# eleurent/rl-agents

Measured on AMD Instinct MI355X. Metric: rollout env-steps/sec (UCT plan(), budget=1000), higher is better.
Workload: dtype f64; 1 GPU; uct_highway_shaped_S10000_A5_budget1000_e33xh30_roots262144_per_gpu; n_roots_per_gpu=262144, n_roots_total=262144, states=10000, actions=5, episodes=33, horizon=30, parallelism=roots sharded over 1 GPU(s)

## Files before the change

### rl_agents_amd/csrc/common.hpp

```cpp
#pragma once
#include <hip/hip_runtime.h>
#include <stdint.h>
#include <stdio.h>
#include <string>
#include <unordered_map>
#include <vector>

#include "../../include/mi355plan.h"
#include "form_names.hpp"

namespace mp {

constexpr int kWave = 64;
constexpr size_t kLdsBytes = 160 * 1024;

extern thread_local std::string g_err;

int fail(int code, const char *fmt, ...);

#define MP_HIP(call)                                                                              \
    do {                                                                                          \
        hipError_t e_ = (call);                                                                   \
        if (e_ != hipSuccess)                                                                     \
            return mp::fail(MP_ERR_HIP, "%s failed: %s (%s:%d)", #call, hipGetErrorString(e_),    \
                            __FILE__, __LINE__);                                                  \
    } while (0)

#define MP_TRY(call)                  \
    do {                              \
        int rc_ = (call);             \
        if (rc_ != MP_OK) return rc_; \
    } while (0)

struct alignas(16) Rec {
    int32_t next;
    uint32_t flags;
    double reward;
};
static_assert(sizeof(Rec) == 16, "Rec must be one dwordx4");

struct DevBuf {
    void *p = nullptr;
    size_t cap = 0;
};

struct TreeMeta {
    int kind = 0;
    int n_roots = 0, A = 0, cap = 0, K = 0, M = 1;
    double gamma = 0.0;
    int buf = 0;
    bool armed = false;
    int il = 0;
    long kept_bound = 0;
    bool virgin = false;
    bool sp = false;
    int n_src = 0;
};

enum { WS_TREE0 = 0, WS_TREE1, WS_TREE2, WS_TREE3, WS_TREE4, WS_TREE5, WS_TREE6, WS_TREE7, WS_IO0, WS_IO1, WS_IO2, WS_IO3, WS_IO4,
       WS_IO5, WS_IO6, WS_IO7, WS_IO8, WS_IO9, WS_TAB0, WS_TAB1, WS_TAB2, WS_TAB3, WS_VI0, WS_VI1, WS_VI2, WS_VI3,
       WS_VI4, WS_VI5, WS_GROOT, WS_JUMP, WS_POL0, WS_POL1, WS_POL2, WS_POL3, WS_POL4,
       WS_IO10,
       WS_COUNT };

struct ViGraphKey {
    const void *model, *T, *R, *term, *Vb, *notclose;
    int iterations, M, S, A, robust, vform;
    double gamma, rtol, atol;
};

}

struct mp_ctx {
    int device = 0;
    hipStream_t stream = nullptr;
    bool own_stream = false;
    hipEvent_t ev0 = nullptr, ev1 = nullptr;
    bool timed = false;
    int n_launches = 0;
    char last_variant[mp::kFormNameBytes] = "";
    hipDeviceProp_t prop;
    mp::DevBuf ws[mp::WS_COUNT];
    mp::TreeMeta tree;
    std::vector<double> tab_host;
    int tab_kind = 0;
    void *vi_graph_exec = nullptr;
    mp::ViGraphKey vi_graph_key;
// ... 249 lines not shown
```

### rl_agents_amd/csrc/uct.hip

```cpp
#include <limits.h>
#include <math.h>
#include <stdlib.h>
#include <string.h>

#include <algorithm>
#include <new>
#include <vector>

#include <type_traits>

#include "common.hpp"
#include "libm_sincos.hpp"
#include "pcg64.hpp"
#include "uct_balance.hpp"
#include "uct_host.hpp"
#include "uct_virgin.hpp"
#include "wave.hpp"

namespace mp {

struct alignas(16) UctNode {
    double value;
    int32_t count;
    int32_t first_child;
// ... 107 lines not shown
    const double temp = (force + polemass_length * (theta_dot * theta_dot) * sintheta) / total_mass;
    const double thetaacc = (c.gravity * sintheta - costheta * temp) /
                            (c.length * (4.0 / 3.0 - c.masspole * (costheta * costheta) / total_mass));
    const double xacc = temp - polemass_length * thetaacc * costheta / total_mass;
    x = x + c.tau * x_dot;
    x_dot = x_dot + c.tau * xacc;
    theta = theta + c.tau * theta_dot;
    theta_dot = theta_dot + c.tau * thetaacc;
    x4[0] = x; x4[1] = x_dot; x4[2] = theta; x4[3] = theta_dot;
    return x < -c.x_threshold || x > c.x_threshold || theta < -c.theta_threshold || theta > c.theta_threshold;
}

__device__ __forceinline__ uint32_t bal_load(const uint32_t *w) { return __hip_atomic_load(w, __ATOMIC_RELAXED, __HIP_MEMORY_SCOPE_WORKGROUP); }
__device__ __forceinline__ void bal_store(uint32_t *w, uint32_t v) { __hip_atomic_store(w, v, __ATOMIC_RELAXED, __HIP_MEMORY_SCOPE_WORKGROUP); }

__device__ __forceinline__ uint32_t simd_id()
{
    uint32_t v;
    asm volatile("s_getreg_b32 %0, hwreg(HW_REG_HW_ID, 4, 2)" : "=s"(v));
    return v;
}
#ifdef MP_WAVE_STAMPS
constexpr int kWaveStampWords = 8;
#endif

enum { ENV_TABLE = 0, ENV_CARTPOLE = 2, ENV_TABLE_LDSR = 3, ENV_TABLE_SPILL = 4 };

#ifndef MP_UCT_MIN_WAVES
#define MP_UCT_MIN_WAVES 1
#endif
#ifndef MP_PCG_WORDS
#define MP_PCG_WORDS 1
#endif
constexpr bool uct_pcg_words_form(int AT, int ENV, bool SP, bool MK, int IL, bool QD)
{
    return ENV != ENV_CARTPOLE && !QD;
}
template <int AT, int ENV, bool SP = false, bool MK = false, int IL = 0, bool QD = false, bool BAL = false>
__global__ __launch_bounds__(ENV == ENV_TABLE_LDSR ? 1024 : (ENV == ENV_CARTPOLE ? 256 : 64),
                             ENV == ENV_TABLE_LDSR ? 1 : (SP && AT > 0 && AT <= 5 && MP_UCT_MIN_WAVES < 4 ? 4 : MP_UCT_MIN_WAVES))
void uct_kernel(UctArgs p)
{
    static_assert(!SP || (AT > 0 && ENV == ENV_TABLE), "per-state policies: table env, |A| known at compile time");
    static_assert(!MK || SP, "listed policies are per-state policies");
    constexpr int NTH = AT > 1 ? AT - 1 : 1;
    constexpr int NQ = (NTH + 1) / 2;
    constexpr int NQ32 = (NTH + 3) / 4;
    constexpr bool LDSR = ENV == ENV_TABLE_LDSR;
    static_assert(!LDSR || (AT > 0 && !SP), "the LDS-resident variant: |A| at compile time, state-independent policies");
    static_assert(!QD || LDSR, "four lanes per root: the LDS-resident model");
    constexpr bool PREG = LDSR || ENV == ENV_TABLE_SPILL;
    constexpr bool CART = ENV == ENV_CARTPOLE;
    constexpr bool RAWU = AT > 0 && !SP;
    constexpr int USH = RAWU ? 0 : 11;
    static_assert(!BAL || (LDSR && !QD), "the wave balance: the one-lane LDS-resident form");
    extern __shared__ __attribute__((aligned(16))) double lds_raw[];
    extern __shared__ __attribute__((aligned(16))) uint32_t lds_bal[];
    double *lds_d = lds_raw + (BAL ? kUctBalBytes / sizeof(double) : 0);
    const int tid = threadIdx.x, lane = tid & 63, wave = tid >> 6;
    const int A = AT > 0 ? AT : p.A, H = p.horizon, E = p.episodes;
    const int nthreads = p.waves * 64;
    double *gpow = lds_d;
    const uint64_t *thr = reinterpret_cast<const uint64_t *>(gpow + (H + 1));
    double *tp = gpow + (H + 1) + A;
    const int TE = p.table_n;
    double *rcp = tp + A;
    double *tpdiv = rcp + (TE + 1);
    const int ntab = (H + 1) + 2 * A + (TE + 1) + A * (TE + 2);
    auto explore = [&](int a, int cnt1) { return cnt1 <= TE + 1 ? tpdiv[a * (TE + 2) + cnt1] : tp[a] / (double)cnt1; };
    auto inv = [&](int c) { return c <= TE ? rcp[c] : 1.0 / (double)c; };
    auto explore_tab = [&](int a, int cnt1) { return tpdiv[a * (TE + 2) + min(cnt1, TE + 1)]; };
// ... 36 lines not shown
        const uint4 *src = reinterpret_cast<const uint4 *>(p.r8);
        uint4 *dst = reinterpret_cast<uint4 *>(r8);
        for (int i = tid; i < n16; i += nthreads) dst[i] = src[i];
    }
    if (LDSR) {
        const int n = p.S * A;
        const int n8 = n >> 3;
        const uint4 *src = reinterpret_cast<const uint4 *>(p.t16);
        uint4 *dst = reinterpret_cast<uint4 *>(t16);
        for (int i = tid; i < n8; i += nthreads) dst[i] = src[i];
        for (int i = (n8 << 3) + tid; i < n; i += nthreads) t16[i] = p.t16[i];
    }
    if constexpr (BAL) {
        const int g0 = blockIdx.x * p.waves + wave;
        const uint32_t mine = (long)g0 * p.lanes < p.n_roots ? uct_bal_word(0, simd_id()) : kUctBalGone;
        if (lane < kUctBalWords && ((lane ^ g0) & (p.waves - 1)) == 0) bal_store(&lds_bal[lane], lane == (g0 & (kUctBalWords - 1)) ? mine : kUctBalGone);
    }
    __syncthreads();
    WAVE_STAMP(1);
    int32_t *path = path_all + wave * 64;
    const int slot = QD ? lane >> 2 : (CART ? lane >> p.rep_shift : lane);
    const bool owner = QD ? (lane & 3) == 0 : true;
    const int r = (blockIdx.x * p.waves + wave) * p.lanes + slot;
#ifdef MP_WAVE_STAMPS
    if (slot >= p.lanes || r >= p.n_roots) { WAVE_STAMP(2); WAVE_STAMP(3); }
#endif
    if (slot >= p.lanes || r >= p.n_roots) return;
    static_assert(IL != 2 || AT > 0, "the group-interleaved layout needs |A| at compile time");
    const TreeRef<IL, AT> tree = tree_of<IL, AT>(p.tree, r, p.cap, A);
    constexpr bool WEXP = IL == 2 && AT > 0 && AT <= 5 && !MK && !LDSR && !CART;
    constexpr int WEXP_PASSES = 4;
    constexpr bool LEAF1 = AT > 0 && !(LDSR && !QD && AT >= 7);
    const bool leaf1 = LEAF1 && p.tree_stores != 0;
    constexpr bool VSKIP = uct_virgin_form(AT, ENV, SP, MK, IL, QD);
    constexpr bool VDEFER = VSKIP && LEAF1;
    const bool vskip = VSKIP && p.tree_stores == 2;
    const bool vdefer = VDEFER && p.tree_stores == 2 && p.n_nodes_in == nullptr;
    bool wave_exp = false;
    if constexpr (WEXP) {
        const int wave_r0 = (blockIdx.x * p.waves + __builtin_amdgcn_readfirstlane(wave)) * 64;
        wave_exp = p.tree_stores != 0 && p.lanes == 64 && wave_r0 + 64 <= p.n_roots;
    }
    const Rec *__restrict__ rec = p.rec;
    Pcg64 g;
    g.load(p.rng + (long)r * 6);
    constexpr bool PCGW = MP_PCG_WORDS != 0 && uct_pcg_words_form(AT, ENV, SP, MK, IL, QD);
    using RollGen = typename std::conditional<PCGW, Pcg64W, Pcg64>::type;
    auto roll_gen = [](const Pcg64 &x) { if constexpr (PCGW) return Pcg64W::from(x); else return x; };
    auto roll_gen_commit = [](Pcg64 &x, const RollGen &y) { if constexpr (PCGW) y.state_to(x); else x = y; };
    uint64_t g4_lo = 0, g4_hi = 0;
    if (QD || (CART && p.rep_shift >= 2)) g.inc_g4(g4_lo, g4_hi);
    uint64_t g16_lo = 0, g16_hi = 0;
    if (CART && p.rep_shift >= 4) g.inc_g16(g16_lo, g16_hi);
    const int32_t s0 = CART ? 0 : p.root_state[r];
    const int32_t st0 = p.root_steps ? p.root_steps[r] : 0;
    const uint32_t done_bit = p.done_on_next ? 2u : 1u;
    const bool root_term = CART ? false : (rec[(long)s0 * A].flags & 1u) != 0;
    double x0[4] = {0.0, 0.0, 0.0, 0.0};
    if (CART) {
#pragma unroll
        for (int i = 0; i < 4; ++i) x0[i] = p.root_x[(long)r * 4 + i];
    }
    const bool cart_flat = CART && p.cp_sincos != SINCOS_DEVICE && p.cp.theta_threshold < 0.8 && !any64(!(fabs(x0[2]) < 0.8));
    int n_nodes = p.n_nodes_in ? p.n_nodes_in[r] : 0;
    constexpr int AR = AT > 0 ? AT : 1;
    constexpr bool RC = AT > 0;
    double tv0 = 0.0, tv[AR];
    int tc0 = 0, tc[AR];
    int tf0 = -1, tf[AR];
// ... 52 lines not shown
            if (pd_ >= 2 + KEEP) hh_ = p.path_spill[(size_t)pd_ * p.spill_stride + r];          \
            out_ = hh_;                                                                         \
        }                                                                                       \
    } while (0)

    constexpr int TREE_PRIO = LDSR && !QD ? 2 : 0;
#ifdef MP_PROFILE
    long long t_sel = 0, t_expd = 0, t_roll = 0, t_bak = 0, n_sel = 0, n_roll = 0;
    const long long t_all0 = clock64();
#define PROF_T(x) const long long x = clock64()
#else
#define PROF_T(x)
#endif
    for (int ep = 0; ep < E; ++ep) {
        PROF_T(c0);
        if constexpr (TREE_PRIO > 0) __builtin_amdgcn_s_setprio(TREE_PRIO);
        int32_t s = s0, st = st0;
        double x4[4] = {x0[0], x0[1], x0[2], x0[3]};
        int node = 0, depth = 0;
        bool terminal = false;
        bool cur_term = root_term;
        double total = 0.0;
        uint32_t cur_mask = mask0;
        if (!RC) PATH_PUT(0, tree.root_handle());
        int hnode = tree.root_handle();
        int fc = RC ? tf0 : tree[0].first_child;
        const bool beyond = RC && any64(tc0 >= TE);
        int node_c = 0;
        while (owner && depth < H && fc >= 0 && !terminal) {
            int act = 0, nfc = -1;
            if (AT > 0) {
                UctNode c[AR];
                bool virgin = false;
                if (fc == 1) {
#pragma unroll
                    for (int a = 0; a < AR; ++a) { c[a].value = tv[a]; c[a].count = tc[a]; c[a].first_child = tf[a]; }
                } else if (VSKIP && vskip && node_c == 1) {
                    virgin = true;
#pragma unroll
                    for (int a = 0; a < AR; ++a) { c[a].value = 0.0; c[a].count = 0; c[a].first_child = -1; }
                } else {
                    UctNode *grp = &tree.child(fc, 0);
#pragma unroll
                    for (int a = 0; a < AR; ++a) c[a] = tree.sibling(grp, a);
                }
                double sc[AR];
                if (SP) {
                    double tpl[AR];
                    if (depth == 0) {
#pragma unroll
                        for (int a = 0; a < AR; ++a) tpl[a] = tp0[a];
                    } else {
                        const double *pr = p.pol_prior + (long)s * p.pol_stride;
                        const double TAk = MK ? p.temperature * (double)__popc(cur_mask) : p.TA;
#pragma unroll
                        for (int a = 0; a < AR; ++a) tpl[a] = TAk * pr[a];
                    }
#pragma unroll
                    for (int a = 0; a < AR; ++a) {
                        sc[a] = c[a].value + tpl[a] / (double)(c[a].count + 1);
                        if (MK && c[a].count < 0) sc[a] = -INFINITY;
                    }
                } else {
                    double ex[AR];
#pragma unroll
                    for (int a = 0; a < AR; ++a) ex[a] = explore_tab(a, c[a].count + 1);
                    if (beyond) {
#pragma nounroll
                        for (int b = 0; b < AR; ++b) {
// ... 9 lines not shown
                    for (int a = 0; a < AR; ++a) sc[a] = c[a].value + ex[a];
                }
                double m = sc[0];
#pragma unroll
                for (int a = 1; a < AR; ++a) m = sc[a] > m ? sc[a] : m;
                int nt = 0;
#pragma unroll
                for (int a = 0; a < AR; ++a) nt += sc[a] == m ? 1 : 0;
                int pick = nt > 1 ? (int)g.below((uint32_t)nt) : 0;
                bool found = false;
                double sel_v = 0.0;
                int sel_c = 0;
#pragma unroll
                for (int a = 0; a < AR; ++a) {
                    const bool eq = sc[a] == m;
                    if (eq && !found && pick == 0) {
                        act = a; nfc = c[a].first_child; found = true;
                        sel_v = c[a].value; sel_c = c[a].count;
                    }
                    if (eq && !found) --pick;
                }
#pragma unroll
                for (int i = 0; i < KEEP; ++i)
                    if (depth + 1 == 2 + i) { kv[i] = sel_v; kc[i] = sel_c; }
                node_c = sel_c;
                if (VDEFER && vdefer && virgin) {
                    UctNode z;
                    z.value = 0.0; z.count = 0; z.first_child = -1;
                    UctNode *grp = &tree.child(fc, 0);
                    const bool deep = depth + 1 >= 2 + KEEP;
#pragma unroll
                    for (int a = 0; a < AR; ++a)
                        if (a != act || deep) tree.sibling(grp, a) = z;
                }
            } else {
                double m = 0.0;
                for (int a = 0; a < A; ++a) {
                    const UctNode c = tree.child(fc, a);
                    const double sc = c.value + explore(a, c.count + 1);
                    if (a == 0 || sc > m) m = sc;
                }
                int nt = 0;
                for (int a = 0; a < A; ++a) {
                    const UctNode c = tree.child(fc, a);
                    nt += (c.value + explore(a, c.count + 1)) == m ? 1 : 0;
                }
                int pick = (int)g.below((uint32_t)nt);
                for (int a = 0; a < A; ++a) {
                    const UctNode c = tree.child(fc, a);
                    if ((c.value + explore(a, c.count + 1)) == m) {
                        if (pick == 0) { act = a; nfc = c.first_child; break; }
                        --pick;
                    }
                }
            }
            const long idx = (long)s * A + act;
            double reward;
            if (CART) {
                terminal = cartpole_step(p.cp, x4, act, p.cp_sincos, sctab);
                reward = 1.0;
            } else if (LDSR) {
                const uint32_t e = t16[idx];
                reward = rdict[r8[idx]];
                const bool next_term = (e & 0x8000u) != 0;
                terminal = p.done_on_next ? next_term : cur_term;
                cur_term = next_term;
// ... 16 lines not shown
            node = fc + act;
            hnode = tree.handle(fc, act);
            ++depth;
            PATH_PUT(depth, hnode);
            fc = nfc;
#ifdef MP_PROFILE
            ++n_sel;
#endif
        }
        PROF_T(c1);
        bool wexp_pend = false;
        if (owner && fc < 0 && depth < H && (!terminal || node == 0)) {
            UctNode n;
            n.value = 0.0; n.count = 0; n.first_child = -1;
            if (RC && node <= A) {
                if (node == 0) tf0 = n_nodes;
#pragma unroll
                for (int a = 0; a < AR; ++a) tf[a] = node == 1 + a ? n_nodes : tf[a];
            } else if (!leaf1) {
                tree.at(hnode).first_child = n_nodes;
            }
            if (LEAF1) fc = n_nodes;
            if (MK) {
                if (node == 0) {
#pragma unroll
                    for (int a = 0; a < AR; ++a) tc[a] = (cur_mask >> a) & 1u ? 0 : -1;
                } else {
                    UctNode *grp = &tree.child(n_nodes, 0);
                    for (int a = 0; a < A; ++a) {
                        n.count = (cur_mask >> a) & 1u ? 0 : -1;
                        tree.sibling(grp, a) = n;
                    }
                }
            } else if (VDEFER && vdefer) {
            } else if (!(RC && node == 0)) {
                if constexpr (WEXP) {
                    wexp_pend = true;
                } else {
                    UctNode *grp = &tree.child(n_nodes, 0);
                    if (AT > 0) {
#pragma unroll
                        for (int a = 0; a < AR; ++a) tree.sibling(grp, a) = n;
                    } else {
                        for (int a = 0; a < A; ++a) tree.sibling(grp, a) = n;
                    }
                }
            }
            n_nodes += A;
        }
        if constexpr (WEXP) {
            UctNode n;
            n.value = 0.0; n.count = 0; n.first_child = -1;
            const int grp_id = n_nodes - AT;
            if (wave_exp) {
                unsigned long long rem = ballot64(wexp_pend);
                for (int pass = 0; pass < WEXP_PASSES && rem != 0ull; ++pass) {
                    const int v = __builtin_amdgcn_readlane(grp_id, __ffsll((long long)rem) - 1);
                    const bool mine = wexp_pend && grp_id == v;
                    const unsigned long long M = ballot64(mine);
                    const uint32_t m_lo = (uint32_t)M, m_hi = (uint32_t)(M >> 32);
                    const int ln = (int)__builtin_amdgcn_mbcnt_hi(~0u, __builtin_amdgcn_mbcnt_lo(~0u, 0u));
                    UctNode *run = tree.base - ln * AT + (unsigned)((v - 1 + AT) << 6);
#pragma nounroll
                    for (int i = 0; i < AT; ++i) {
                        const unsigned e = (unsigned)(i * 64 + ln), q = e / (unsigned)AT;
                        if ((((q & 32u) ? m_hi : m_lo) >> (q & 31u)) & 1u) run[e] = n;
                    }
// ... 556 lines not shown
                    n -= tree.handle(1, 0);
                    double v = tv[0];
                    int cnt = tc[0];
#pragma unroll
                    for (int a = 1; a < AR; ++a) { v = n == a ? tv[a] : v; cnt = n == a ? tc[a] : cnt; }
                    cnt += 1;
                    v += inv_fast(cnt) * (total - v);
#pragma unroll
                    for (int a = 0; a < AR; ++a) { tv[a] = n == a ? v : tv[a]; tc[a] = n == a ? cnt : tc[a]; }
                }
                tc0 += 1;
                tv0 += inv_fast(tc0) * (total - tv0);
            }
        }
#ifdef MP_PROFILE
        { const long long c4 = clock64(); t_sel += c1 - c0; t_expd += c2 - c1; t_roll += c3 - c2; t_bak += c4 - c3; }
#endif
    }
    if constexpr (BAL) {
        if ((((uint32_t)r) & 63u) == 0u) bal_store(&lds_bal[((uint32_t)r >> 6) & (kUctBalWords - 1)], kUctBalGone);
    }
    WAVE_STAMP(2);
    if constexpr (TREE_PRIO > 0) __builtin_amdgcn_s_setprio(0);
#ifdef MP_PROFILE
    if (r == 0)
        printf("uct prof wave0: total=%lld select=%lld expand=%lld rollout=%lld backup=%lld | lane0 select steps=%lld rollout steps=%lld\n",
               (long long)(clock64() - t_all0), t_sel, t_expd, t_roll, t_bak, n_sel, n_roll);
#endif
    if (!owner) return;
    if (CART && (lane & ((1 << p.rep_shift) - 1)) != 0) return;
    if (RC) {
        UctNode w;
        w.value = tv0; w.count = tc0; w.first_child = tf0;
        tree[0] = w;
        if (tf0 == 1) {
#pragma unroll
            for (int a = 0; a < AR; ++a) {
                w.value = tv[a]; w.count = tc[a]; w.first_child = tf[a];
                tree.child(1, a) = w;
            }
        }
    }
    g.store(p.rng + (long)r * 6);
    {
        int len = 0;
        int fc = tree[0].first_child;
        int at_c = 0;
        while (fc >= 0) {
            if (VDEFER && vdefer && at_c == 1) {
                if (p.plans && len < p.max_plan_len) p.plans[(long)r * p.max_plan_len + len] = 0;
                ++len;
                break;
            }
            int mc = tree.child(fc, 0).count;
            for (int a = 1; a < A; ++a) mc = max(mc, tree.child(fc, a).count);
            int best = -1;
            double bv = 0.0;
            for (int a = 0; a < A; ++a) {
                const UctNode c = tree.child(fc, a);
                if (c.count == mc && (best < 0 || c.value > bv)) { best = a; bv = c.value; }
            }
            if (p.plans && len < p.max_plan_len) p.plans[(long)r * p.max_plan_len + len] = best;
            ++len;
            at_c = tree.child(fc, best).count;
            fc = tree.child(fc, best).first_child;
        }
        if (p.plans)
            for (int i = len; i < p.max_plan_len; ++i) p.plans[(long)r * p.max_plan_len + i] = -1;
        if (p.plan_len) p.plan_len[r] = len;
    }
    if (p.n_nodes_out) p.n_nodes_out[r] = n_nodes;
    if (p.root_value) p.root_value[r] = tree[0].value;
    if (p.env_steps) p.env_steps[r] = (int64_t)steps_taken;
    const int rfc = tree[0].first_child;
    for (int a = 0; a < A; ++a) {
        if (p.root_child_count) p.root_child_count[(long)r * A + a] = rfc >= 0 ? max(tree.child(rfc, a).count, 0) : 0;
        if (p.root_child_value) p.root_child_value[(long)r * A + a] = rfc >= 0 ? tree.child(rfc, a).value : 0.0;
    }
    WAVE_STAMP(3);
#undef WAVE_STAMP
}

template <int AT, bool EACH = false, bool MW = false>
__global__ __launch_bounds__(EACH ? 256 : 1024, EACH ? 4 : 1) void uct_lone_kernel(UctArgs p)
{
    static_assert(!(EACH && MW), "one MDP per root is staged per workgroup: one root each");
    static_assert(AT >= 2 && AT <= 8, "|A| with a compile-time specialisation");
    constexpr int A = AT, NTH = AT - 1;
    extern __shared__ __attribute__((aligned(16))) double lds_d[];
    const int tid = threadIdx.x, lane = tid & 63, nthreads = blockDim.x;
    const int H = p.horizon, E = p.episodes, TE = p.table_n;
    double *gpow = lds_d;
    double *tp = gpow + (H + 1) + A;
    double *rcp = tp + A;
    double *tpdiv = rcp + (TE + 1);
    const int ntab = (H + 1) + 2 * A + (TE + 1) + A * (TE + 2);
    const int ntab2 = (ntab + 1) & ~1;
    const int SA = (EACH ? p.Sb : p.S) * A;
    const double *rdict = lds_d + ntab2;
    double *rew = lds_d + ntab2;
    uint16_t *t16 = EACH ? reinterpret_cast<uint16_t *>(rew + ((SA + 1) & ~1))
                         : reinterpret_cast<uint16_t *>(lds_d + ntab2 + (MW ? 0 : ((p.n_rdict + 1) & ~1)));
    uint8_t *r8 = reinterpret_cast<uint8_t *>(t16 + ((SA + 7) & ~7));
    uint32_t *jump0 = (EACH || MW) ? reinterpret_cast<uint32_t *>(r8) : reinterpret_cast<uint32_t *>(r8 + ((SA + 15) & ~15));
    const int W = MW ? p.waves : 1;
    const int wstride = ((H + 5) * 8 + p.cap * 6 + 3) & ~3;
    uint32_t *jump = jump0 + (MW ? (tid >> 6 < W ? tid >> 6 : 0) * wstride : 0);
// ... 629 lines not shown
            int mc = tnode[fc].count;
            for (int a = 1; a < A; ++a) mc = max(mc, tnode[fc + a].count);
            int best = -1;
            double bv = 0.0;
            for (int a = 0; a < A; ++a) {
                const UctNode c = tnode[fc + a];
                if (c.count == mc && (best < 0 || c.value > bv)) { best = a; bv = c.value; }
            }
            if (p.plans && len < p.max_plan_len) p.plans[(long)r * p.max_plan_len + len] = best;
            ++len;
            fc = tnode[fc + best].first_child;
        }
        if (p.plans)
            for (int i = len; i < p.max_plan_len; ++i) p.plans[(long)r * p.max_plan_len + i] = -1;
        if (p.plan_len) p.plan_len[r] = len;
        if (p.n_nodes_out) p.n_nodes_out[r] = n_nodes;
        if (p.root_value) p.root_value[r] = tnode[0].value;
        if (p.env_steps) p.env_steps[r] = (int64_t)steps_taken;
        const int rfc = tnode[0].first_child;
        for (int a = 0; a < A; ++a) {
            if (p.root_child_count) p.root_child_count[(long)r * A + a] = rfc >= 0 ? max(tnode[rfc + a].count, 0) : 0;
            if (p.root_child_value) p.root_child_value[(long)r * A + a] = rfc >= 0 ? tnode[rfc + a].value : 0.0;
        }
    }
}

template <int IL>
__global__ void uct_path_count_kernel(UctNode *trees, int root, int cap, int A, const int32_t *actions, int n, int64_t *out, int virgin)
{
    const TreeRef<IL, 0> tree = tree_of<IL, 0>(trees, root, cap, A);
    int node = 0;
    bool unstored = false;
    for (int i = 0; i < n; ++i) {
        const int fc = unstored ? -1 : tree[node].first_child;
        const int a = actions[i];
        if (fc < 0 || a < 0 || a >= A) { out[0] = -1; return; }
        unstored = virgin && tree[node].count == 1;
        node = fc + a;
    }
    const int c = unstored ? 0 : tree[node].count;
    out[0] = c < 0 ? -1 : c;
}

template <int IL>
__global__ __launch_bounds__(64) void uct_reroot_kernel(int n_roots, int n_src, int A, int cap_old, int cap_new,
                                                        const UctNode *__restrict__ old_trees, UctNode *__restrict__ new_trees,
                                                        const int32_t *n_old, const int32_t *__restrict__ source,
                                                        const int32_t *__restrict__ actions,
                                                        int32_t *n_new,
                                                        int virgin)
{
    const int r = blockIdx.x * blockDim.x + threadIdx.x;
    if (r >= n_roots) return;
    const int q = source ? source[r] : r;
    if (q < 0 || q >= n_src) {
        n_new[r] = 0;
        return;
    }
    const TreeRef<IL, 0> o = tree_of<IL, 0>(const_cast<UctNode *>(old_trees), q, cap_old, A);
    const TreeRef<IL, 0> n = tree_of<IL, 0>(new_trees, r, cap_new, A);
    const int a = actions[r];
    if (n_old[q] < 1 || o[0].first_child < 0 || a < 0 || a >= A || o[o[0].first_child + a].count < 0) {
        n_new[r] = 0;
        return;
    }
    int head = 0, tail = 1;
    UctNode first;
    first.first_child = o[0].first_child + a;
    n[0] = first;
    while (head < tail) {
        const int oid = n[head].first_child;
        UctNode src;
        src.value = 0.0; src.count = 0; src.first_child = -1;
        if (oid >= 0) src = o[oid];
        UctNode out;
        out.value = src.value; out.count = src.count; out.first_child = -1;
        if (src.first_child >= 0) {
            out.first_child = tail;
            const bool unstored = virgin && src.count == 1;
            for (int c = 0; c < A; ++c) {
                UctNode q;
                q.value = 0.0; q.count = 0; q.first_child = unstored ? -2 : src.first_child + c;
                n[tail + c] = q;
            }
            tail += A;
        }
        n[head] = out;
        ++head;
    }
    n_new[r] = tail;
}

struct PolBuild {
    int S, A, stride, frq, rows, shift, can_pack;
    const double *prior, *rollout;
    const uint8_t *listed, *slot;
    const Rec *rec;
    double *hp;
    uint64_t *ht;
    uint32_t *lmask;
    uint32_t *hf, *hfr, *hp16;
    int32_t *err;
};
__device__ __forceinline__ void pol_err(const PolBuild &b, int code, int s)
{
    if (atomicCAS(b.err, 0, code) == 0) b.err[1] = s;
}
__global__ void policy_rows_kernel(PolBuild b)
{
    const int s = blockIdx.x * blockDim.x + threadIdx.x;
    if (s >= b.S) return;
    const int A = b.A, r = s % b.rows;
    double cdf[8];
    double acc = 0.0;
    unsigned seen = 0;
// ... 38 lines not shown
        const uint64_t hi = t53 >> b.shift;
        f[4 + a] = hi > 0xffffffffULL ? 0xffffffffu : (uint32_t)hi;
        if (b.can_pack && a < 4) th[a] = (t53 >> 43) > 1023ULL ? 1023u : (uint32_t)(t53 >> 43);
    }
    if (b.can_pack) {
        uint32_t *g = b.hp16 + (size_t)i * 4;
        g[0] = (uint32_t)nx | (th[0] << 20);
        g[1] = (rc.y & 3u) | (th[1] << 2) | (th[2] << 12) | (th[3] << 22);
        g[2] = rc.z; g[3] = rc.w;
    }
}
__global__ void policy_froll_kernel(PolBuild b)
{
    const long i = (long)blockIdx.x * blockDim.x + threadIdx.x;
    if (i >= (long)b.S * b.A) return;
    const int s = (int)(i / b.A), k = (int)(i % b.A), r = s % b.rows;
    const int c = b.slot[(size_t)r * b.A + k];
    if (c >= b.A) return;
    const uint4 *src = reinterpret_cast<const uint4 *>(b.hf) + ((size_t)s * b.A + c) * b.frq;
    uint4 *dst = reinterpret_cast<uint4 *>(b.hfr) + (size_t)i * b.frq;
    for (int q = 0; q < b.frq; ++q) dst[q] = src[q];
}

}

using namespace mp;

static int uct_reroot_now(mp_ctx *ctx, long cap_new)
{
    const int n_roots = ctx->tree.n_roots;
    const int old_slot = ctx->tree.buf ? WS_TREE2 : WS_TREE0, new_slot = ctx->tree.buf ? WS_TREE0 : WS_TREE2;
    UctNode *nw = nullptr;
    MP_TRY(ws_get(ctx, new_slot, (size_t)((n_roots + 63) & ~63) * tree_stride_alloc(ctx->tree.il, cap_new, ctx->tree.A), &nw));
    const int virgin = ctx->tree.virgin ? 1 : 0;
    ctx->tree.virgin = false;
    return reroot_apply(ctx, cap_new, [&](const Reroot &r) {
        hipLaunchKernelGGL(ctx->tree.il == 2 ? uct_reroot_kernel<2> : uct_reroot_kernel<0>, dim3((unsigned)((r.n_roots + 63) / 64)), dim3(64), 0,
                           ctx->stream, r.n_roots, r.n_src, r.A, r.cap_old, r.cap_new, (const UctNode *)ctx->ws[old_slot].p, nw, r.sizes, r.src,
                           r.acts, r.sizes_new, virgin);
    });
}

enum UctForm { UF_GLOBAL, UF_GLOBAL_SPILL, UF_LDSR, UF_QUAD, UF_LONE, UF_LONE_MW, UF_LONE_EACH, UF_ROW_EACH, UF_ROW_SHARED,
               UF_CARTPOLE, UF_POLICY, UF_COUNT };
static_assert(UF_COUNT == kUctForms, "uct_form_name (form_names.hpp) names the forms in this order");

constexpr int kUnset = INT_MIN;
struct UctKnobs {
    int model;
    int quad, lone, each, row, rows;
    int lone_waves;
    int row_waves, row_roots, lanes, cart_rep, cart_waves;
    int path;
    long ldsr_waves;
    int tree_stores;
    int balance;
};
static int uct_knob(const char *name)
{
    const char *e = getenv(name);
    return e ? atoi(e) : kUnset;
}
static UctKnobs uct_knobs_read()
{
    UctKnobs k;
    const char *model = getenv("MP_UCT_MODEL"), *path = getenv("MP_UCT_PATH"), *ldsr_waves = getenv("MP_UCT_LDSR_WAVES");
    k.model = model ? !strcmp(model, "ldsr") : kUnset;
    k.path = path ? path[0] == 's' : kUnset;
    k.ldsr_waves = ldsr_waves ? atol(ldsr_waves) : LONG_MIN;
    k.quad = uct_knob("MP_UCT_QUAD"); k.lone = uct_knob("MP_UCT_LONE"); k.each = uct_knob("MP_UCT_EACH");
    k.row = uct_knob("MP_UCT_ROW"); k.rows = uct_knob("MP_UCT_ROWS");
    k.lone_waves = uct_knob("MP_UCT_LONE_WAVES");
    if (k.lone_waves != kUnset && k.lone_waves != 1 && k.lone_waves != 2 && k.lone_waves != 4 && k.lone_waves != 8) k.lone_waves = 0;
    k.row_waves = uct_knob("MP_UCT_ROW_WAVES"); k.row_roots = uct_knob("MP_UCT_ROW_ROOTS"); k.lanes = uct_knob("MP_UCT_LANES");
    k.cart_rep = uct_knob("MP_UCT_CART_REP"); k.cart_waves = uct_knob("MP_UCT_CART_WAVES");
    const char *tree_stores = getenv("MP_UCT_TREE_STORES");
    k.tree_stores = tree_stores && !strcmp(tree_stores, "lane") ? 0 : (tree_stores && !strcmp(tree_stores, "group") ? 1 : 2);
    k.balance = uct_knob("MP_UCT_BALANCE") != 0;
    return k;
}

struct UctCall {
    int n_roots, episodes, horizon, A, S, NB, Sb;
    bool t16, r8;
    int n_rdict;
    bool cart, pol, listed;
    int kept_il;
    int cus;
};
struct UctChoice {
    UctForm form;
    int tree_il, lanes, waves, rep_shift, roots_per_wg, threads;
    size_t lds;
};

static int uct_choose(const UctCall &c, const UctKnobs &k, UctChoice *out)
{
    const int A = c.A, H = c.horizon, E = c.episodes;
    const long n = c.n_roots, cus = c.cus > 0 ? c.cus : 256, cap = 1 + (long)E * A;
    const bool at_known = A >= 2 && A <= 8, fresh = c.kept_il < 0, forced = k.model != kUnset;
    const int te_max = (int)(16384 / (sizeof(double) * (size_t)(A + 1))), TE = E < te_max ? E : te_max;
    const size_t ntab = (size_t)(H + 1) + 2 * (size_t)A + (TE + 1) + (size_t)A * (TE + 2), tabs = ntab * sizeof(double);
    auto dbl16 = [](size_t m) { return ((m + 1) & ~(size_t)1) * sizeof(double); };
    auto t16_bytes = [](size_t m) { return ((m + 7) & ~(size_t)7) * 2; };
    const size_t sa = (size_t)c.S * A, sa_each = (size_t)(c.NB > 1 && c.Sb > 0 ? c.Sb : c.S) * A;
    const size_t jump = (size_t)(H + 5) * 32, path_stack = (size_t)(H + 1) * 64 * sizeof(int32_t);
    const size_t tree_lds = (size_t)cap * (sizeof(UctNode) + sizeof(double)) + (size_t)(H + 1) * sizeof(int32_t) + 16;
    const size_t lds_ldsr = dbl16(ntab) + dbl16(c.n_rdict) + t16_bytes(sa) + ((sa + 15) & ~(size_t)15);
    const size_t lds_quad = lds_ldsr + jump, lds_lone = lds_quad + tree_lds;
    const size_t lds_each = dbl16(ntab) + dbl16(sa_each) + t16_bytes(sa_each) + jump + tree_lds;
// ... 84 lines not shown
            return fail(MP_ERR_ARG, "mp_uct_plan: horizon %d / episodes %d need %zu B of LDS tables (> 64 KiB)", H, E, o.lds);
        if (o.lds > 64 * 1024 || (k.path == 1 && !fallback && !c.pol)) {
            o.form = UF_GLOBAL_SPILL;
            o.lds = tabs;
        }
        break;
    }
    if (o.form != UF_LONE && o.form != UF_LONE_MW && o.form != UF_LONE_EACH && o.form != UF_ROW_EACH && o.form != UF_ROW_SHARED) {
        o.roots_per_wg = o.waves * o.lanes;
        o.threads = o.waves * 64;
    }
    if (c.pol && !c.cart && !at_known)
        return fail(MP_ERR_ARG, "mp_uct_plan_policy: |A| = %d is not in 2..8: per-state policies over more actions plan through "
                                "mp_uct_plan_stochastic_policy (it takes deterministic tables too)", A);
    *out = o;
    return MP_OK;
}

template <typename Kernel>
static int uct_go(Kernel kernel, const UctChoice &ch, const UctArgs &a, hipStream_t st)
{
    const size_t lds = ch.lds + (a.balance ? (size_t)kUctBalBytes : 0);
    if (lds > 64 * 1024)
        MP_HIP(hipFuncSetAttribute(reinterpret_cast<const void *>(kernel), hipFuncAttributeMaxDynamicSharedMemorySize, (int)lds));
    hipLaunchKernelGGL(kernel, dim3((unsigned)((a.n_roots + ch.roots_per_wg - 1) / ch.roots_per_wg)), dim3((unsigned)ch.threads), lds,
                       st, a);
    return MP_OK;
}

template <int AT>
static int uct_launch(const UctChoice &ch, bool listed, const UctArgs &a, hipStream_t st)
{
    const bool il2 = a.tree_il == 2;
    if constexpr (AT > 0) {
        switch (ch.form) {
        case UF_LDSR:
            if constexpr (uct_balance_form(AT))
                if (a.balance) return uct_go(uct_kernel<AT, ENV_TABLE_LDSR, false, false, 2, false, true>, ch, a, st);
            return uct_go(uct_kernel<AT, ENV_TABLE_LDSR, false, false, 2>, ch, a, st);
        case UF_QUAD: return uct_go(uct_kernel<AT, ENV_TABLE_LDSR, false, false, 2, true>, ch, a, st);
        case UF_LONE: return uct_go(uct_lone_kernel<AT>, ch, a, st);
        case UF_LONE_MW: return uct_go(uct_lone_kernel<AT, false, true>, ch, a, st);
        case UF_LONE_EACH: return uct_go(uct_lone_kernel<AT, true>, ch, a, st);
        case UF_ROW_EACH: return uct_go(uct_row_kernel<AT>, ch, a, st);
        case UF_ROW_SHARED: return uct_go(uct_row_kernel<AT, true>, ch, a, st);
        case UF_POLICY:
            if (listed)
                return il2 ? uct_go(uct_kernel<AT, ENV_TABLE, true, true, 2>, ch, a, st) : uct_go(uct_kernel<AT, ENV_TABLE, true, true, 0>, ch, a, st);
            return il2 ? uct_go(uct_kernel<AT, ENV_TABLE, true, false, 2>, ch, a, st) : uct_go(uct_kernel<AT, ENV_TABLE, true, false, 0>, ch, a, st);
        case UF_GLOBAL:
            if (il2) return uct_go(uct_kernel<AT, ENV_TABLE, false, false, 2>, ch, a, st);
            break;
        case UF_GLOBAL_SPILL:
            if (il2) return uct_go(uct_kernel<AT, ENV_TABLE_SPILL, false, false, 2>, ch, a, st);
            break;
        default: break;
        }
    }
    if constexpr (AT == 2)
        if (ch.form == UF_CARTPOLE) return uct_go(uct_kernel<2, ENV_CARTPOLE>, ch, a, st);
    if (ch.form == UF_GLOBAL && !il2) return uct_go(uct_kernel<AT, ENV_TABLE>, ch, a, st);
    if (ch.form == UF_GLOBAL_SPILL && !il2) return uct_go(uct_kernel<AT, ENV_TABLE_SPILL>, ch, a, st);
    return fail(MP_ERR_ARG, "mp_uct_plan: no %s kernel for |A| = %d in tree layout %d", uct_form_name(ch.form).c_str(), a.A, a.tree_il);
}

static int uct_dispatch(const UctChoice &ch, bool listed, const UctArgs &a, hipStream_t st)
{
    static int (*const launch[8])(const UctChoice &, bool, const UctArgs &, hipStream_t) = {
        uct_launch<2>, uct_launch<3>, uct_launch<4>, uct_launch<5>, uct_launch<6>, uct_launch<7>, uct_launch<8>, uct_launch<0>};
    return launch[a.A >= 2 && a.A <= 8 ? a.A - 2 : 7](ch, listed, a, st);
}


static int uct_check(const mp_ctx *ctx, const UctPlan &c)
{
    const mp_model *model = c.model;
    const mp_policy *pol = c.pol;
    if (!ctx || !model || !c.root_state || !c.rng_state || (!pol && (!c.prior_p || !c.rollout_p)))
        return fail(MP_ERR_ARG, "mp_uct_plan: NULL argument");
    const bool cart = model->mode == MP_MODE_CARTPOLE;
    if (pol && !cart && pol->model == model && pol->model_serial == model->serial && pol->ctx == ctx && !pol->frec && pol->A > 8)
        return fail(MP_ERR_ARG, "mp_uct_plan_policy: |A| = %d is not in 2..8: per-state policies over more actions plan through "
                                "mp_uct_plan_stochastic_policy (it takes deterministic tables too)", pol->A);
    if (pol && (cart || pol->model != model || pol->model_serial != model->serial || pol->ctx != ctx || !pol->frec))
        return fail(MP_ERR_ARG, "mp_uct_plan_policy: the policy was not loaded for this model");
    if (model->mode != MP_MODE_DETERMINISTIC && !cart)
// ... 107 lines not shown
    const UctForm form = ch->form;
    if (form == UF_QUAD || form == UF_LONE || form == UF_LONE_MW || form == UF_LONE_EACH || form == UF_ROW_EACH || form == UF_ROW_SHARED ||
        form == UF_CARTPOLE)
        MP_TRY(uct_jump_table(ctx, c.horizon, &a->jump));
    return MP_OK;
}

static int uct_trees(mp_ctx *ctx, const UctPlan &c, bool cont, const UctChoice &ch, UctArgs *a)
{
    const int n_roots = c.n_roots, A = a->A, H = c.horizon, E = c.episodes;
    long cap_use = 1 + (long)E * A;
    a->n_nodes_in = nullptr;
    if (cont) {
        cap_use = uct_kept_cap(ctx, H, E, A);
        MP_TRY(uct_reroot_now(ctx, cap_use));
        MP_TRY(ws_get(ctx, WS_TREE1, (size_t)n_roots, &a->n_nodes_out));
        a->tree = (UctNode *)ctx->ws[ctx->tree.buf ? WS_TREE2 : WS_TREE0].p;
        a->n_nodes_in = a->n_nodes_out;
    } else {
        MP_TRY(ws_get(ctx, WS_TREE1, (size_t)n_roots, &a->n_nodes_out));
        uct_fresh_tree(ctx, H, E, A);
        ctx->tree.il = ch.tree_il;
        MP_TRY(ws_get(ctx, WS_TREE0, (size_t)((n_roots + 63) & ~63) * tree_stride_alloc(ctx->tree.il, cap_use, A), &a->tree));
    }
    a->cap = (int)cap_use;
    a->tree_il = ctx->tree.il;
    a->path_spill = nullptr; a->spill_stride = 0;
    if (ch.form == UF_LDSR || ch.form == UF_QUAD || ch.form == UF_GLOBAL_SPILL) {
        a->spill_stride = ((long)n_roots + 63) & ~63L;
        MP_TRY(ws_get(ctx, WS_TREE4, (size_t)(H + 1) * (size_t)a->spill_stride, &a->path_spill));
    }
    ctx->tree.kind = 1; ctx->tree.n_roots = n_roots; ctx->tree.A = A; ctx->tree.cap = (int)cap_use;
    const int env = ch.form == UF_LDSR ? ENV_TABLE_LDSR : (ch.form == UF_GLOBAL ? ENV_TABLE : (ch.form == UF_GLOBAL_SPILL ? ENV_TABLE_SPILL : -1));
    ctx->tree.virgin = !cont && a->tree_stores == 2 && env >= 0 &&
                       uct_virgin_form(A, env, false, false, ctx->tree.il, false);
    return MP_OK;
}

static int uct_stage(mp_ctx *ctx, WaveIo *io, bool *all_pinned)
{
    *all_pinned = false;
    if (io->mem == MP_MEM_HOST) {
        void *alias[10];
        bool all = true;
        for (int i = 0; i < io->n; ++i) {
            const WaveIo::Item &t = io->item[i];
            alias[i] = t.host && t.mem == MP_MEM_HOST ? pinned_alias(ctx, t.host, io->bytes(t)) : t.host;
            if (t.host && !alias[i]) all = false;
        }
        *all_pinned = all;
        long zc_max = 65536;
        if (const char *e = getenv("MP_ZERO_COPY_MAX")) zc_max = atol(e);
        if (all && !getenv("MP_NO_ZERO_COPY") && io->n_roots <= zc_max) {
            for (int i = 0; i < io->n; ++i) { io->item[i].host = alias[i]; io->item[i].mem = MP_MEM_DEVICE; }
            io->mem = MP_MEM_DEVICE; io->rmem = MP_MEM_DEVICE;
        }
    }
    for (int i = 0; i < io->n; ++i) {
        WaveIo::Item &t = io->item[i];
        void *d = t.host;
        if (t.mem == MP_MEM_HOST && t.host) MP_TRY(ws_reserve(ctx, t.slot, io->bytes(t), &d));
        t.base = static_cast<char *>(d);
    }
    return MP_OK;
}

static int uct_run_chunk(const WaveIo &io, const UctChoice &ch, bool listed, UctArgs &a, int r0, int r1, hipStream_t s)
{
// ... 494 lines not shown
}

int mp_uct_tree_capacity(mp_ctx *ctx, int32_t *cap)
{
    if (!ctx || !cap) return fail(MP_ERR_ARG, "mp_uct_tree_capacity: NULL argument");
    if (ctx->tree.kind != 1) return fail(MP_ERR_ARG, "mp_uct_tree_capacity: no UCT tree on this ctx");
    *cap = ctx->tree.cap;
    return MP_OK;
}

int mp_uct_reset_tree(mp_ctx *ctx)
{
    if (!ctx) return fail(MP_ERR_ARG, "ctx is NULL");
    if (selection_pending(ctx)) ctx->tree.n_roots = ctx->tree.n_src;
    ctx->tree.armed = false;
    ctx->tree.n_src = 0;
    return MP_OK;
}

int mp_uct_path_count(mp_ctx *ctx, int32_t root, const int32_t *actions, int32_t n, int64_t *count)
{
    if (!ctx || !count || (n > 0 && !actions)) return fail(MP_ERR_ARG, "mp_uct_path_count: NULL argument");
    if (ctx->tree.kind != 1) return fail(MP_ERR_ARG, "mp_uct_path_count: no UCT tree on this ctx");
    if (root < 0 || root >= ctx->tree.n_roots || n < 0) return fail(MP_ERR_ARG, "mp_uct_path_count: root %d / length %d out of range", root, n);
    if (selection_pending(ctx)) return fail(MP_ERR_ARG, "mp_uct_path_count: a selection of the trees is armed: plan (or mp_uct_reset_tree) first");
    MP_HIP(hipSetDevice(ctx->device));
    hipStream_t st = ctx->stream;
    UctNode *trees = (UctNode *)ctx->ws[ctx->tree.buf ? WS_TREE2 : WS_TREE0].p;
    int32_t *d_act = nullptr;
    int64_t *d_out = nullptr;
    MP_TRY(ws_get(ctx, WS_IO1, (size_t)(n > 0 ? n : 1), &d_act));
    MP_TRY(ws_get(ctx, WS_IO8, 1, &d_out));
    if (n > 0) MP_HIP(hipMemcpyAsync(d_act, actions, (size_t)n * sizeof(int32_t), hipMemcpyHostToDevice, st));
    const int tcap = ctx->tree.cap, A = ctx->tree.A, virgin = ctx->tree.virgin ? 1 : 0;
    if (ctx->tree.il == 2) hipLaunchKernelGGL(uct_path_count_kernel<2>, dim3(1), dim3(1), 0, st, trees, root, tcap, A, d_act, n, d_out, virgin);
    else hipLaunchKernelGGL(uct_path_count_kernel<0>, dim3(1), dim3(1), 0, st, trees, root, tcap, A, d_act, n, d_out, virgin);
    MP_HIP(hipGetLastError());
    MP_HIP(hipMemcpyAsync(count, d_out, sizeof(int64_t), hipMemcpyDeviceToHost, st));
    MP_HIP(hipStreamSynchronize(st));
    return MP_OK;
}

int mp_uct_tree_export(mp_ctx *ctx, int32_t root, int32_t cap, int32_t *n_nodes, int32_t *parent, int32_t *action,
                       int64_t *count, double *value, int32_t *first_child, int32_t *n_children)
{
    if (!ctx) return fail(MP_ERR_ARG, "ctx is NULL");
    if (ctx->tree.kind != 1) return fail(MP_ERR_ARG, "mp_uct_tree_export: no UCT tree on this ctx");
    if (root < 0 || root >= ctx->tree.n_roots) return fail(MP_ERR_ARG, "mp_uct_tree_export: root %d out of range", root);
    if (selection_pending(ctx)) return fail(MP_ERR_ARG, "mp_uct_tree_export: a selection of the trees is armed: plan (or mp_uct_reset_tree) first");
    const int tcap = ctx->tree.cap, A = ctx->tree.A;
    std::vector<UctNode> h((size_t)tcap);
    MP_HIP(hipSetDevice(ctx->device));
    MP_HIP(hipStreamSynchronize(ctx->stream));
    const UctNode *trees = (const UctNode *)ctx->ws[ctx->tree.buf ? WS_TREE2 : WS_TREE0].p;
    if (ctx->tree.il == 2) {
        const int groups = (tcap - 1) / A + 1;
        std::vector<UctNode> g((size_t)groups * A);
        MP_HIP(hipMemcpy2D(g.data(), (size_t)A * sizeof(UctNode), trees + ((long)(root >> 6) * (tcap + A) * 64 + (long)(root & 63) * A),
                           (size_t)64 * A * sizeof(UctNode), (size_t)A * sizeof(UctNode), (size_t)groups, hipMemcpyDeviceToHost));
        for (int i = 0; i < tcap; ++i) h[i] = g[(size_t)(i + A - 1)];
    } else
        MP_HIP(hipMemcpy(h.data(), trees + (long)root * tcap, (size_t)tcap * sizeof(UctNode), hipMemcpyDeviceToHost));
    const int n = uct_virgin_fill(h.data(), tcap, A, ctx->tree.virgin);
    std::vector<int32_t> id((size_t)n, -1);
    int kept = 0;
    for (int i = 0; i < n; ++i)
        if (h[i].count >= 0) id[i] = kept++;
// ... 27 lines not shown
```

### rl_agents_amd/csrc/uct_virgin.hpp

```cpp
#pragma once

namespace mp {

constexpr bool uct_virgin_form(int AT, int ENV, bool SP, bool MK, int IL, bool QD)
{
    return IL == 2 && !SP && !MK && !QD && AT >= 2 && AT <= 5 && (ENV == 3 || ENV == 0 || ENV == 4);
}

template <typename Node>
inline int uct_virgin_fill(Node *h, int tcap, int A, bool virgin)
{
    int n = 1;
    for (int i = 0; i < n && i < tcap; ++i) {
        const int fc = h[i].first_child;
        if (fc < 0) continue;
        if (virgin && h[i].count == 1)
            for (int a = 0; a < A && fc + a < tcap; ++a) { h[fc + a].value = 0.0; h[fc + a].count = 0; h[fc + a].first_child = -1; }
        if (fc + A > n) n = fc + A;
    }
    return n;
}

}
```

Before: 262.6 billion env-steps/s.

## Track stored children with a visited bitmask packed into first_child

Adds a new default tree-store mode that packs a per-child 'stored' bitmask into the high bits of each node's first_child word. Selection skips loading child nodes that were never written, and expansion no longer zero-fills whole sibling groups; only the chosen child gets written on its first visit. The aim is to cut global memory loads and stores during tree descent and expansion. In exchange, every reader of the tree (plan extraction, export, reroot, path count) must decode the mask, and the child index is limited to 24 bits.

```diff
diff --git a/rl_agents_amd/csrc/common.hpp b/rl_agents_amd/csrc/common.hpp
--- a/rl_agents_amd/csrc/common.hpp
+++ b/rl_agents_amd/csrc/common.hpp
@@ -52,7 +52,7 @@
     bool armed = false;
     int il = 0;
     long kept_bound = 0;
-    bool virgin = false;
+    int virgin = 0;
     bool sp = false;
     int n_src = 0;
 };
diff --git a/rl_agents_amd/csrc/uct.hip b/rl_agents_amd/csrc/uct.hip
--- a/rl_agents_amd/csrc/uct.hip
+++ b/rl_agents_amd/csrc/uct.hip
@@ -163,11 +163,14 @@
 #ifndef MP_PCG_WORDS
 #define MP_PCG_WORDS 1
 #endif
+#ifndef MP_UCT_MASK_LOADS
+#define MP_UCT_MASK_LOADS 1
+#endif
 constexpr bool uct_pcg_words_form(int AT, int ENV, bool SP, bool MK, int IL, bool QD)
 {
     return ENV != ENV_CARTPOLE && !QD;
 }
-template <int AT, int ENV, bool SP = false, bool MK = false, int IL = 0, bool QD = false, bool BAL = false>
+template <int AT, int ENV, bool SP = false, bool MK = false, int IL = 0, bool QD = false, bool BAL = false, bool VM = false>
 __global__ __launch_bounds__(ENV == ENV_TABLE_LDSR ? 1024 : (ENV == ENV_CARTPOLE ? 256 : 64),
                              ENV == ENV_TABLE_LDSR ? 1 : (SP && AT > 0 && AT <= 5 && MP_UCT_MIN_WAVES < 4 ? 4 : MP_UCT_MIN_WAVES))
 void uct_kernel(UctArgs p)
@@ -270,9 +273,11 @@
     constexpr int WEXP_PASSES = 4;
     constexpr bool LEAF1 = AT > 0 && !(LDSR && !QD && AT >= 7);
     const bool leaf1 = LEAF1 && p.tree_stores != 0;
-    constexpr bool VSKIP = uct_virgin_form(AT, ENV, SP, MK, IL, QD);
+    static_assert(!VM || (uct_mask_form(AT, ENV, SP, MK, IL, QD) && LEAF1 && !CART), "the visited mask: the forms of uct_mask_form");
+    constexpr bool VMASK = VM;
+    constexpr bool VSKIP = !VM && uct_virgin_form(AT, ENV, SP, MK, IL, QD);
     constexpr bool VDEFER = VSKIP && LEAF1;
-    const bool vskip = VSKIP && p.tree_stores == 2;
+    const bool vskip = VSKIP && p.tree_stores >= 2;
     const bool vdefer = VDEFER && p.tree_stores == 2 && p.n_nodes_in == nullptr;
     bool wave_exp = false;
     if constexpr (WEXP) {
@@ -391,9 +396,27 @@
             if (AT > 0) {
                 UctNode c[AR];
                 bool virgin = false;
+                const int fcw = fc;
+                if (VMASK) fc &= kUctChildBits;
                 if (fc == 1) {
 #pragma unroll
                     for (int a = 0; a < AR; ++a) { c[a].value = tv[a]; c[a].count = tc[a]; c[a].first_child = tf[a]; }
+                } else if (VMASK) {
+                    UctNode *grp = &tree.child(fc, 0);
+#pragma unroll
+                    for (int a = 0; a < AR; ++a) {
+                        const bool stored = ((fcw >> (kUctMaskShift + a)) & 1) != 0;
+                        c[a].value = 0.0; c[a].count = 0; c[a].first_child = -1;
+#if MP_UCT_MASK_LOADS
+                        if (stored) c[a] = tree.sibling(grp, a);
+#else
+                        if ((fcw >> kUctMaskShift) != 0) {
+                            const UctNode ld = tree.sibling(grp, a);
+                            asm volatile("" ::"v"(ld.count));
+                            if (stored) c[a] = ld;
+                        }
+#endif
+                    }
                 } else if (VSKIP && vskip && node_c == 1) {
                     virgin = true;
 #pragma unroll
@@ -469,6 +492,20 @@
 #pragma unroll
                     for (int a = 0; a < AR; ++a)
                         if (a != act || deep) tree.sibling(grp, a) = z;
+                }
+                if (VMASK && depth >= 1 && !((fcw >> (kUctMaskShift + act)) & 1)) {
+                    const int w = fcw | (1 << (kUctMaskShift + act));
+                    if (depth == 1) {
+#pragma unroll
+                        for (int a = 0; a < AR; ++a) tf[a] = node == 1 + a ? w : tf[a];
+                    } else {
+                        tree.at(hnode).first_child = w;
+                    }
+                    if (depth + 1 >= 2 + KEEP) {
+                        UctNode z;
+                        z.value = 0.0; z.count = 0; z.first_child = -1;
+                        tree.child(fc, act) = z;
+                    }
                 }
             } else {
                 double m = 0.0;
@@ -551,7 +588,7 @@
                         tree.sibling(grp, a) = n;
                     }
                 }
-            } else if (VDEFER && vdefer) {
+            } else if ((VDEFER && vdefer) || VMASK) {
             } else if (!(RC && node == 0)) {
                 if constexpr (WEXP) {
                     wexp_pend = true;
@@ -1174,6 +1211,7 @@
     if (RC) {
         UctNode w;
         w.value = tv0; w.count = tc0; w.first_child = tf0;
+        if (VMASK && tf0 >= 0) w.first_child = tf0 | (((1 << AR) - 1) << kUctMaskShift);
         tree[0] = w;
         if (tf0 == 1) {
 #pragma unroll
@@ -1194,18 +1232,27 @@
                 ++len;
                 break;
             }
-            int mc = tree.child(fc, 0).count;
-            for (int a = 1; a < A; ++a) mc = max(mc, tree.child(fc, a).count);
+            unsigned stored = ~0u;
+            if (VMASK) { stored = (unsigned)fc >> kUctMaskShift; fc &= kUctChildBits; }
+            auto child = [&](int a) {
+                UctNode c;
+                c.value = 0.0; c.count = 0; c.first_child = -1;
+                if (!VMASK || ((stored >> a) & 1u)) c = tree.child(fc, a);
+                return c;
+            };
+            int mc = child(0).count;
+            for (int a = 1; a < A; ++a) mc = max(mc, child(a).count);
             int best = -1;
             double bv = 0.0;
             for (int a = 0; a < A; ++a) {
-                const UctNode c = tree.child(fc, a);
+                const UctNode c = child(a);
                 if (c.count == mc && (best < 0 || c.value > bv)) { best = a; bv = c.value; }
             }
             if (p.plans && len < p.max_plan_len) p.plans[(long)r * p.max_plan_len + len] = best;
             ++len;
-            at_c = tree.child(fc, best).count;
-            fc = tree.child(fc, best).first_child;
+            const UctNode b = child(best);
+            at_c = b.count;
+            fc = b.first_child;
         }
         if (p.plans)
             for (int i = len; i < p.max_plan_len; ++i) p.plans[(long)r * p.max_plan_len + i] = -1;
@@ -1214,7 +1261,8 @@
     if (p.n_nodes_out) p.n_nodes_out[r] = n_nodes;
     if (p.root_value) p.root_value[r] = tree[0].value;
     if (p.env_steps) p.env_steps[r] = (int64_t)steps_taken;
-    const int rfc = tree[0].first_child;
+    int rfc = tree[0].first_child;
+    if (VMASK) rfc = uct_word_child(rfc);
     for (int a = 0; a < A; ++a) {
         if (p.root_child_count) p.root_child_count[(long)r * A + a] = rfc >= 0 ? max(tree.child(rfc, a).count, 0) : 0;
         if (p.root_child_value) p.root_child_value[(long)r * A + a] = rfc >= 0 ? tree.child(rfc, a).value : 0.0;
@@ -1910,10 +1958,11 @@
     int node = 0;
     bool unstored = false;
     for (int i = 0; i < n; ++i) {
-        const int fc = unstored ? -1 : tree[node].first_child;
+        const int w = unstored ? -1 : tree[node].first_child;
+        const int fc = virgin == kUctTreeMasked ? uct_word_child(w) : w;
         const int a = actions[i];
         if (fc < 0 || a < 0 || a >= A) { out[0] = -1; return; }
-        unstored = virgin && tree[node].count == 1;
+        unstored = virgin == kUctTreeMasked ? !uct_word_stored(w, a) : (virgin == kUctTreeCount1 && tree[node].count == 1);
         node = fc + a;
     }
     const int c = unstored ? 0 : tree[node].count;
@@ -1938,13 +1987,14 @@
     const TreeRef<IL, 0> o = tree_of<IL, 0>(const_cast<UctNode *>(old_trees), q, cap_old, A);
     const TreeRef<IL, 0> n = tree_of<IL, 0>(new_trees, r, cap_new, A);
     const int a = actions[r];
-    if (n_old[q] < 1 || o[0].first_child < 0 || a < 0 || a >= A || o[o[0].first_child + a].count < 0) {
+    const int rfc = n_old[q] < 1 ? -1 : (virgin == kUctTreeMasked ? uct_word_child(o[0].first_child) : o[0].first_child);
+    if (rfc < 0 || a < 0 || a >= A || o[rfc + a].count < 0) {
         n_new[r] = 0;
         return;
     }
     int head = 0, tail = 1;
     UctNode first;
-    first.first_child = o[0].first_child + a;
+    first.first_child = rfc + a;
     n[0] = first;
     while (head < tail) {
         const int oid = n[head].first_child;
@@ -1955,10 +2005,12 @@
         out.value = src.value; out.count = src.count; out.first_child = -1;
         if (src.first_child >= 0) {
             out.first_child = tail;
-            const bool unstored = virgin && src.count == 1;
+            const int sfc = virgin == kUctTreeMasked ? uct_word_child(src.first_child) : src.first_child;
             for (int c = 0; c < A; ++c) {
+                const bool unstored = virgin == kUctTreeMasked ? !uct_word_stored(src.first_child, c)
+                                                               : (virgin == kUctTreeCount1 && src.count == 1);
                 UctNode q;
-                q.value = 0.0; q.count = 0; q.first_child = unstored ? -2 : src.first_child + c;
+                q.value = 0.0; q.count = 0; q.first_child = unstored ? -2 : sfc + c;
                 n[tail + c] = q;
             }
             tail += A;
@@ -2063,8 +2115,8 @@
     const int old_slot = ctx->tree.buf ? WS_TREE2 : WS_TREE0, new_slot = ctx->tree.buf ? WS_TREE0 : WS_TREE2;
     UctNode *nw = nullptr;
     MP_TRY(ws_get(ctx, new_slot, (size_t)((n_roots + 63) & ~63) * tree_stride_alloc(ctx->tree.il, cap_new, ctx->tree.A), &nw));
-    const int virgin = ctx->tree.virgin ? 1 : 0;
-    ctx->tree.virgin = false;
+    const int virgin = ctx->tree.virgin;
+    ctx->tree.virgin = kUctTreeWhole;
     return reroot_apply(ctx, cap_new, [&](const Reroot &r) {
         hipLaunchKernelGGL(ctx->tree.il == 2 ? uct_reroot_kernel<2> : uct_reroot_kernel<0>, dim3((unsigned)((r.n_roots + 63) / 64)), dim3(64), 0,
                            ctx->stream, r.n_roots, r.n_src, r.A, r.cap_old, r.cap_new, (const UctNode *)ctx->ws[old_slot].p, nw, r.sizes, r.src,
@@ -2106,7 +2158,7 @@
     k.row_waves = uct_knob("MP_UCT_ROW_WAVES"); k.row_roots = uct_knob("MP_UCT_ROW_ROOTS"); k.lanes = uct_knob("MP_UCT_LANES");
     k.cart_rep = uct_knob("MP_UCT_CART_REP"); k.cart_waves = uct_knob("MP_UCT_CART_WAVES");
     const char *tree_stores = getenv("MP_UCT_TREE_STORES");
-    k.tree_stores = tree_stores && !strcmp(tree_stores, "lane") ? 0 : (tree_stores && !strcmp(tree_stores, "group") ? 1 : 2);
+    k.tree_stores = !tree_stores ? 3 : (!strcmp(tree_stores, "lane") ? 0 : (!strcmp(tree_stores, "group") ? 1 : (!strcmp(tree_stores, "virgin") ? 2 : 3)));
     k.balance = uct_knob("MP_UCT_BALANCE") != 0;
     return k;
 }
@@ -2257,9 +2309,16 @@
 static int uct_launch(const UctChoice &ch, bool listed, const UctArgs &a, hipStream_t st)
 {
     const bool il2 = a.tree_il == 2;
+    [[maybe_unused]] const bool vm = a.tree_stores == 3;
     if constexpr (AT > 0) {
         switch (ch.form) {
         case UF_LDSR:
+            if constexpr (uct_mask_form(AT, ENV_TABLE_LDSR, false, false, 2, false))
+                if (vm) {
+                    if constexpr (uct_balance_form(AT))
+                        if (a.balance) return uct_go(uct_kernel<AT, ENV_TABLE_LDSR, false, false, 2, false, true, true>, ch, a, st);
+                    return uct_go(uct_kernel<AT, ENV_TABLE_LDSR, false, false, 2, false, false, true>, ch, a, st);
+                }
             if constexpr (uct_balance_form(AT))
                 if (a.balance) return uct_go(uct_kernel<AT, ENV_TABLE_LDSR, false, false, 2, false, true>, ch, a, st);
             return uct_go(uct_kernel<AT, ENV_TABLE_LDSR, false, false, 2>, ch, a, st);
@@ -2274,9 +2333,13 @@
                 return il2 ? uct_go(uct_kernel<AT, ENV_TABLE, true, true, 2>, ch, a, st) : uct_go(uct_kernel<AT, ENV_TABLE, true, true, 0>, ch, a, st);
             return il2 ? uct_go(uct_kernel<AT, ENV_TABLE, true, false, 2>, ch, a, st) : uct_go(uct_kernel<AT, ENV_TABLE, true, false, 0>, ch, a, st);
         case UF_GLOBAL:
+            if constexpr (uct_mask_form(AT, ENV_TABLE, false, false, 2, false))
+                if (il2 && vm) return uct_go(uct_kernel<AT, ENV_TABLE, false, false, 2, false, false, true>, ch, a, st);
             if (il2) return uct_go(uct_kernel<AT, ENV_TABLE, false, false, 2>, ch, a, st);
             break;
         case UF_GLOBAL_SPILL:
+            if constexpr (uct_mask_form(AT, ENV_TABLE_SPILL, false, false, 2, false))
+                if (il2 && vm) return uct_go(uct_kernel<AT, ENV_TABLE_SPILL, false, false, 2, false, false, true>, ch, a, st);
             if (il2) return uct_go(uct_kernel<AT, ENV_TABLE_SPILL, false, false, 2>, ch, a, st);
             break;
         default: break;
@@ -2450,8 +2513,11 @@
     }
     ctx->tree.kind = 1; ctx->tree.n_roots = n_roots; ctx->tree.A = A; ctx->tree.cap = (int)cap_use;
     const int env = ch.form == UF_LDSR ? ENV_TABLE_LDSR : (ch.form == UF_GLOBAL ? ENV_TABLE : (ch.form == UF_GLOBAL_SPILL ? ENV_TABLE_SPILL : -1));
-    ctx->tree.virgin = !cont && a->tree_stores == 2 && env >= 0 &&
-                       uct_virgin_form(A, env, false, false, ctx->tree.il, false);
+    if (a->tree_stores == 3 && !(!cont && env >= 0 && uct_mask_form(A, env, false, false, ctx->tree.il, false) && cap_use <= kUctChildBits))
+        a->tree_stores = 2;
+    ctx->tree.virgin = kUctTreeWhole;
+    if (!cont && env >= 0 && a->tree_stores == 3) ctx->tree.virgin = kUctTreeMasked;
+    else if (!cont && env >= 0 && a->tree_stores == 2 && uct_virgin_form(A, env, false, false, ctx->tree.il, false)) ctx->tree.virgin = kUctTreeCount1;
     return MP_OK;
 }
 
@@ -3012,7 +3078,7 @@
     MP_TRY(ws_get(ctx, WS_IO1, (size_t)(n > 0 ? n : 1), &d_act));
     MP_TRY(ws_get(ctx, WS_IO8, 1, &d_out));
     if (n > 0) MP_HIP(hipMemcpyAsync(d_act, actions, (size_t)n * sizeof(int32_t), hipMemcpyHostToDevice, st));
-    const int tcap = ctx->tree.cap, A = ctx->tree.A, virgin = ctx->tree.virgin ? 1 : 0;
+    const int tcap = ctx->tree.cap, A = ctx->tree.A, virgin = ctx->tree.virgin;
     if (ctx->tree.il == 2) hipLaunchKernelGGL(uct_path_count_kernel<2>, dim3(1), dim3(1), 0, st, trees, root, tcap, A, d_act, n, d_out, virgin);
     else hipLaunchKernelGGL(uct_path_count_kernel<0>, dim3(1), dim3(1), 0, st, trees, root, tcap, A, d_act, n, d_out, virgin);
     MP_HIP(hipGetLastError());
diff --git a/rl_agents_amd/csrc/uct_virgin.hpp b/rl_agents_amd/csrc/uct_virgin.hpp
--- a/rl_agents_amd/csrc/uct_virgin.hpp
+++ b/rl_agents_amd/csrc/uct_virgin.hpp
@@ -1,21 +1,39 @@
 #pragma once
 
 namespace mp {
+
+enum UctTreeMode { kUctTreeWhole = 0, kUctTreeCount1 = 1, kUctTreeMasked = 2 };
+
+constexpr int kUctMaskShift = 24;
+constexpr int kUctChildBits = (1 << kUctMaskShift) - 1;
+
+constexpr int uct_word_child(int w) { return w < 0 ? -1 : w & kUctChildBits; }
+constexpr unsigned uct_word_mask(int w) { return w < 0 ? 0u : (unsigned)w >> kUctMaskShift; }
+constexpr bool uct_word_stored(int w, int a) { return ((uct_word_mask(w) >> a) & 1u) != 0u; }
 
 constexpr bool uct_virgin_form(int AT, int ENV, bool SP, bool MK, int IL, bool QD)
 {
     return IL == 2 && !SP && !MK && !QD && AT >= 2 && AT <= 5 && (ENV == 3 || ENV == 0 || ENV == 4);
 }
 
+constexpr bool uct_mask_form(int AT, int ENV, bool SP, bool MK, int IL, bool QD)
+{
+    return uct_virgin_form(AT, ENV, SP, MK, IL, QD);
+}
+
 template <typename Node>
-inline int uct_virgin_fill(Node *h, int tcap, int A, bool virgin)
+inline int uct_virgin_fill(Node *h, int tcap, int A, int mode)
 {
     int n = 1;
     for (int i = 0; i < n && i < tcap; ++i) {
-        const int fc = h[i].first_child;
-        if (fc < 0) continue;
-        if (virgin && h[i].count == 1)
-            for (int a = 0; a < A && fc + a < tcap; ++a) { h[fc + a].value = 0.0; h[fc + a].count = 0; h[fc + a].first_child = -1; }
+        const int w = h[i].first_child;
+        if (w < 0) continue;
+        const int fc = mode == kUctTreeMasked ? uct_word_child(w) : w;
+        h[i].first_child = fc;
+        for (int a = 0; a < A && fc + a < tcap; ++a) {
+            const bool unstored = mode == kUctTreeMasked ? !uct_word_stored(w, a) : (mode == kUctTreeCount1 && h[i].count == 1);
+            if (unstored) { h[fc + a].value = 0.0; h[fc + a].count = 0; h[fc + a].first_child = -1; }
+        }
         if (fc + A > n) n = fc + A;
     }
     return n;
```

Result: faster. 267.9 billion env-steps/s (median of 6 runs) (+2.0%).
